# Ophiase/Stochastic-Vector-Oracle-Consensus

Measured on AMD Instinct MI355X. Metric: consensus updates/sec (N oracles x D dims, batched), higher is better.
Workload: dtype fp32; 1 GPU; model=svoc-consensus N=256 D=4096 streaming (f=32, constrained), global_batch=1024, seq_len=4096, parallelism=dp1, engine_mode=fast, storage=fp32, n_oracles=256, dimension=4096, n_failing=32, hip_graph=True, backend_world=1, stream_pool=89, independent_failing=False, transactional=False, fast_transactional=True, pipeline_chunks=2

## Files before the change

### csrc/include/svoc/slabdma.hpp

```cpp
#pragma once

#include <hip/hip_runtime.h>
#include <stdint.h>

#include "svoc/bufload.hpp"

namespace svoc {

typedef uint32_t u32x32_t __attribute__((ext_vector_type(32)));
typedef uint32_t u32x4_t __attribute__((ext_vector_type(4)));
struct RawRows {
  u32x32_t lo, hi;
  SVOC_DEV uint32_t at(int i) const { return i < 32 ? lo[i] : hi[i - 32]; }
};

template <int NSEG>
struct SlabDma {
  static constexpr int P = 64 / NSEG, CPR = P / 4, RPI = 64 / CPR;
  int vlane;
  int row0;
  int colb;
  SVOC_DEV SlabDma(int lane, int rowb) {
    const int j = lane / CPR;
    row0 = (j % NSEG) * 64 + j / NSEG;
    colb = (lane % CPR) * 16;
    vlane = row0 * rowb + colb;
  }
  SVOC_DEV int row_of(int k) const { return row0 + k * (RPI / NSEG); }
  static SVOC_DEV uint32_t lds_addr(uint32_t* region) {
    return (uint32_t)(uintptr_t)(__attribute__((address_space(3))) void*)region;
  }
  SVOC_DEV void issue(const BufDesc& rs, uint32_t* region, int rowb, int col0) const {
    const int vo = vlane + col0 * 4;
    const uint32_t lds0 = lds_addr(region);
#pragma unroll
    for (int k = 0; k < 16; ++k) {
      const uint32_t lds = lds0 + k * 1024u;
      int keep;
      asm volatile(
          "s_mov_b32 %0, m0\n\t"
          "s_mov_b32 m0, %3\n\t"
          "s_nop 0\n\t"
          "buffer_load_dwordx4 %1, %2, %4 offen lds\n\t"
          "s_mov_b32 m0, %0"
          : "=&s"(keep)
          : "v"(vo), "s"(rs.w), "s"(lds), "s"(k * (RPI / NSEG) * rowb)
          : "memory");
    }
  }
  template <class Sel, class OffB>
  SVOC_DEV void issue_mapped(const BufDesc& rs, const BufDesc& rb, uint32_t* region, int rowb, int col0, Sel sel,
                             OffB off_b) const {
    const int vo = vlane + col0 * 4;
    const uint32_t lds0 = lds_addr(region);
#pragma unroll
    for (int k = 0; k < 16; ++k) {
      const uint32_t lds = lds0 + k * 1024u;
      const uint32_t fb = sel(k);
      const int vb = off_b(k, fb);
      int keep;
      uint64_t sx;
      asm volatile(
          "s_mov_b32 %0, m0\n\t"
          "s_mov_b32 m0, %7\n\t"
          "s_mov_b64 %1, exec\n\t"
          "v_cmp_ne_u32 vcc, 0, %4\n\t"
          "s_nop 4\n\t"
          "s_andn2_b64 exec, %1, vcc\n\t"
          "s_nop 0\n\t"
          "buffer_load_dwordx4 %2, %5, %8 offen lds\n\t"
          "s_and_b64 exec, %1, vcc\n\t"
          "s_nop 0\n\t"
          "buffer_load_dwordx4 %3, %6, 0 offen lds\n\t"
          "s_mov_b64 exec, %1\n\t"
          "s_mov_b32 m0, %0"
          : "=&s"(keep), "=&s"(sx)
          : "v"(vo), "v"(vb), "v"(fb), "s"(rs.w), "s"(rb.w), "s"(lds), "s"(k * (RPI / NSEG) * rowb)
          : "vcc", "memory");
    }
  }
  template <class Sel, class OffB>
  SVOC_DEV void issue_mapped3(const BufDesc& rs, const BufDesc& rb, const BufDesc& rp, uint32_t* region, int rowb,
                              int col0, Sel sel, OffB off_b) const {
    const int vo = vlane + col0 * 4;
    const uint32_t lds0 = lds_addr(region);
#pragma unroll
    for (int k = 0; k < 16; ++k) {
      const uint32_t lds = lds0 + k * 1024u;
      const int fb = sel(k);
      const int vb = off_b(k);
      int keep;
      uint64_t sx, sp;
      asm volatile(
          "s_mov_b32 %0, m0\n\t"
          "s_mov_b32 m0, %9\n\t"
          "s_mov_b64 %1, exec\n\t"
          "v_cmp_gt_i32_e64 %2, 0, %5\n\t"
          "v_cmp_lt_i32 vcc, 0, %5\n\t"
          "s_nop 4\n\t"
          "s_and_b64 exec, %1, vcc\n\t"
          "s_nop 0\n\t"
          "buffer_load_dwordx4 %4, %7, 0 offen lds\n\t"
          "s_and_b64 exec, %1, %2\n\t"
          "s_or_b64 vcc, vcc, %2\n\t"
          "buffer_load_dwordx4 %4, %8, 0 offen lds\n\t"
          "s_andn2_b64 exec, %1, vcc\n\t"
          "s_nop 0\n\t"
          "buffer_load_dwordx4 %3, %6, %10 offen lds\n\t"
          "s_mov_b64 exec, %1\n\t"
          "s_mov_b32 m0, %0"
          : "=&s"(keep), "=&s"(sx), "=&s"(sp)
          : "v"(vo), "v"(vb), "v"(fb), "s"(rs.w), "s"(rb.w), "s"(rp.w), "s"(lds), "s"(k * (RPI / NSEG) * rowb)
          : "vcc", "memory");
    }
  }
};

}
```

### csrc/include/svoc/sortnet.hpp

```cpp
#pragma once

#include <hip/hip_runtime.h>
#include <stdint.h>

namespace svoc {

typedef unsigned short u16x2 __attribute__((ext_vector_type(2)));
typedef short s16x2 __attribute__((ext_vector_type(2)));

#define SVOC_DEV __device__ __forceinline__

SVOC_DEV u16x2 kmin(u16x2 a, u16x2 b) { return __builtin_elementwise_min(a, b); }
SVOC_DEV u16x2 kmax(u16x2 a, u16x2 b) { return __builtin_elementwise_max(a, b); }
SVOC_DEV uint32_t as_u32(u16x2 v) { return __builtin_bit_cast(uint32_t, v); }
SVOC_DEV u16x2 as_k(uint32_t v) { return __builtin_bit_cast(u16x2, v); }
SVOC_DEV uint32_t kmin(uint32_t a, uint32_t b) { return a < b ? a : b; }
SVOC_DEV uint32_t kmax(uint32_t a, uint32_t b) { return a < b ? b : a; }
SVOC_DEV uint32_t as_u32(uint32_t v) { return v; }
template <class K>
SVOC_DEV K key_from(uint32_t v) { return __builtin_bit_cast(K, v); }

SVOC_DEV u16x2 bf16x2_to_key(uint32_t raw) {
  u16x2 r = as_k(raw);
  u16x2 s = __builtin_bit_cast(u16x2, __builtin_bit_cast(s16x2, r) >> (short)15);
// ... 176 lines not shown
  m = 0u - (uint32_t)((k >> 4) & 1);
#pragma unroll
  for (int j = 0; j < 2; ++j) a[j] = blend(a[2 * j], a[2 * j + 1], m);
  m = 0u - (uint32_t)((k >> 5) & 1);
  return as_k(blend(a[0], a[1], m));
}

template <int NSEG, int P>
SVOC_DEV u16x2 group_select(const u16x2 (&r)[64], int rank, int lane) {
  const u16x2 v = reg_select(r, rank & 63);
  if constexpr (NSEG == 1) {
    return v;
  } else {
    const int owner = (rank >> 6) * P + (lane % P);
    return shfl_k(v, owner);
  }
}

template <int NSEG, int P, class K>
SVOC_DEV void middle_pair(const K (&r)[64], int seg, int lane, K& lo, K& hi) {
  if constexpr (NSEG == 1) {
    lo = r[31];
    hi = r[32];
  } else {
    constexpr int h = NSEG / 2;
    const int pw = lane % P;
    lo = shfl_k(r[63], (h - 1) * P + pw);
    hi = shfl_k(r[0], h * P + pw);
  }
}

template <int XM>
SVOC_DEV void xswap(uint32_t& x, uint32_t& y) {
  static_assert(XM == 16 || XM == 32, "lane-half exchange distance");
  if constexpr (XM == 32) {
    const auto t = __builtin_amdgcn_permlane32_swap(x, y, false, false);
    x = t[0];
    y = t[1];
  } else {
    const auto t = __builtin_amdgcn_permlane16_swap(x, y, false, false);
    x = t[0];
    y = t[1];
  }
}

template <int XM, class K>
SVOC_DEV void xhc_swap(K (&r)[64]) {
#pragma unroll
  for (int k = 0; k < 32; ++k) {
    uint32_t x = as_u32(r[2 * k]), y = as_u32(r[2 * k + 1]);
    xswap<XM>(x, y);
    y = ~y;
    const K lo = kmin(key_from<K>(x), key_from<K>(y)), hi = kmax(key_from<K>(x), key_from<K>(y));
    x = as_u32(lo);
    y = as_u32(hi);
    xswap<XM>(x, y);
    r[2 * k] = key_from<K>(x);
    r[2 * k + 1] = key_from<K>(y);
  }
}

template <int XM, class K>
SVOC_DEV void xhc_middle(const K (&r)[64], K& mx, K& mn) {
  mx = key_from<K>(0u);
  mn = key_from<K>(0xffffffffu);
#pragma unroll
  for (int k = 0; k < 32; ++k) {
    uint32_t x = as_u32(r[2 * k]), y = as_u32(r[2 * k + 1]);
    xswap<XM>(x, y);
    y = ~y;
    mx = kmax(mx, kmin(key_from<K>(x), key_from<K>(y)));
    mn = kmin(mn, kmax(key_from<K>(x), key_from<K>(y)));
  }
}

template <int NSEG>
SVOC_DEV uint32_t group_polarity(int seg) {
  if constexpr (NSEG == 2) return seg == 1 ? 0xffffffffu : 0u;
  else if constexpr (NSEG == 4) return (seg == 1 || seg == 2) ? 0xffffffffu : 0u;
  else return 0u;
}

template <int NSEG, class K>
SVOC_DEV void median_group(K (&r)[64], K& lo, K& hi) {
  sort_oem<64>(r);
  if constexpr (NSEG == 1) {
    lo = r[31];
    hi = r[32];
  } else {
    if constexpr (NSEG == 4) {
      xhc_swap<16>(r);
      merge64(r);
    }
    K mx, mn;
    xhc_middle<32>(r, mx, mn);
#pragma unroll
    for (int m = 16; m <= 32; m <<= 1) {
      if (NSEG == 2 && m == 16) continue;
      mx = kmax(mx, shfl_xor_k(mx, m));
      mn = kmin(mn, shfl_xor_k(mn, m));
    }
    lo = mx;
    hi = mn;
  }
}

template <int NSEG, int P, class K>
SVOC_DEV void median_group_wide(K (&r)[64], int seg, int lane, K& lo, K& hi) {
  static_assert(NSEG == 8 || NSEG == 16 || NSEG == 32 || NSEG == 64, "wide groups");
  sort_group<NSEG, P>(r, seg);
  middle_pair<NSEG, P>(r, seg, lane, lo, hi);
}


template <int XM, class K>
SVOC_DEV void xhc_pol(K (&r)[64], uint32_t iy, uint32_t ox, uint32_t oy) {
#pragma unroll
  for (int k = 0; k < 32; ++k) {
    uint32_t x = as_u32(r[2 * k]), y = as_u32(r[2 * k + 1]);
    xswap<XM>(x, y);
    y ^= iy;
    const K lo = kmin(key_from<K>(x), key_from<K>(y)), hi = kmax(key_from<K>(x), key_from<K>(y));
    x = as_u32(lo) ^ ox;
    y = as_u32(hi) ^ oy;
    xswap<XM>(x, y);
    r[2 * k] = key_from<K>(x);
    r[2 * k + 1] = key_from<K>(y);
  }
}

template <int H, class K>
SVOC_DEV void bitonic_top(const K (&r)[64], K (&out)[H]) {
  constexpr int KT = H - 1;
  static_assert(KT >= 2 && KT <= 32 && (KT & (KT - 1)) == 0, "H = 2^k + 1, at most 33");
  K t[64];
#pragma unroll
  for (int i = 0; i < 64; ++i) t[i] = r[i];
#pragma unroll
  for (int n = 64; n > 2 * KT; n >>= 1) {
#pragma unroll
    for (int i = 0; i < n / 2; ++i) t[i] = kmax(t[i], t[i + n / 2]);
  }
  K mx = kmin(t[0], t[KT]);
#pragma unroll
  for (int i = 0; i < KT; ++i) {
    const K a = t[i], b = t[i + KT];
    if (i) mx = kmax(mx, kmin(a, b));
    t[i] = kmax(a, b);
  }
#pragma unroll
  for (int j = KT / 2; j > 0; j >>= 1) {
#pragma unroll
    for (int i = 0; i < KT; ++i) {
      const int l = i ^ j;
      if (l > i) {
        const K a = t[i], b = t[l];
        t[i] = kmin(a, b);
        t[l] = kmax(a, b);
      }
    }
  }
  out[0] = mx;
#pragma unroll
  for (int i = 0; i < KT; ++i) out[i + 1] = t[i];
}

template <int NSEG, int P, int H, class K>
SVOC_DEV void window_group(K (&r)[64], int seg, int lane, K (&w)[NSEG == 1 ? 2 * H : H], K& lo, K& hi) {
  sort_oem<64>(r);
  if constexpr (NSEG == 1) {
#pragma unroll
    for (int m = 0; m < H; ++m) {
      w[m] = r[32 - H + m];
      w[H + m] = ~r[32 + H - 1 - m];
    }
    lo = r[31];
    hi = r[32];
  } else {
    if constexpr (NSEG == 2) {
      xhc_pol<32>(r, ~0u, 0u, ~0u);
    } else {
      xhc_swap<16>(r);
      merge64(r);
      xhc_pol<32>(r, ~0u, 0u, 0u);
      const uint32_t xm = seg >= 2 ? ~0u : 0u;
      xhc_pol<16>(r, 0u, xm, xm);
    }
    bitonic_top<H>(r, w);
    constexpr int slo = NSEG == 2 ? 0 : 1;
    const int pw = lane % P;
    lo = shfl_k(w[H - 1], slo * P + pw);
    hi = ~shfl_k(w[H - 1], (slo + 1) * P + pw);
  }
}



template <int XM, int L, class K>
SVOC_DEV void xhc_swap_n(K (&r)[L]) {
#pragma unroll
  for (int k = 0; k < L / 2; ++k) {
    uint32_t x = as_u32(r[2 * k]), y = as_u32(r[2 * k + 1]);
    xswap<XM>(x, y);
    y = ~y;
    const K lo = kmin(key_from<K>(x), key_from<K>(y)), hi = kmax(key_from<K>(x), key_from<K>(y));
    x = as_u32(lo);
    y = as_u32(hi);
    xswap<XM>(x, y);
    r[2 * k] = key_from<K>(x);
    r[2 * k + 1] = key_from<K>(y);
  }
}
template <int XM, int L, class K>
SVOC_DEV void xhc_pol_n(K (&r)[L], uint32_t iy, uint32_t ox, uint32_t oy) {
#pragma unroll
  for (int k = 0; k < L / 2; ++k) {
    uint32_t x = as_u32(r[2 * k]), y = as_u32(r[2 * k + 1]);
    xswap<XM>(x, y);
    y ^= iy;
    const K lo = kmin(key_from<K>(x), key_from<K>(y)), hi = kmax(key_from<K>(x), key_from<K>(y));
    x = as_u32(lo) ^ ox;
    y = as_u32(hi) ^ oy;
    xswap<XM>(x, y);
    r[2 * k] = key_from<K>(x);
    r[2 * k + 1] = key_from<K>(y);
  }
}
template <int L, class K>
SVOC_DEV void merge_n(K (&r)[L]) {
#pragma unroll
  for (int j = L / 2; j > 0; j >>= 1) {
#pragma unroll
    for (int i = 0; i < L; ++i) {
      const int l = i ^ j;
      if (l > i) {
        const K a = r[i], b = r[l];
        r[i] = kmin(a, b);
        r[l] = kmax(a, b);
      }
    }
  }
}
template <int H, int L, class K>
SVOC_DEV void bitonic_top_n(const K (&r)[L], K (&out)[H]) {
  constexpr int KT = H - 1;
  static_assert(2 * KT == L, "bitonic_top_n: L = 2 (H - 1)");
  K t[KT];
  K mx = kmin(r[0], r[KT]);
#pragma unroll
  for (int i = 0; i < KT; ++i) {
    const K a = r[i], b = r[i + KT];
    if (i) mx = kmax(mx, kmin(a, b));
    t[i] = kmax(a, b);
  }
#pragma unroll
  for (int j = KT / 2; j > 0; j >>= 1) {
#pragma unroll
    for (int i = 0; i < KT; ++i) {
      const int l = i ^ j;
      if (l > i) {
        const K a = t[i], b = t[l];
        t[i] = kmin(a, b);
        t[l] = kmax(a, b);
      }
    }
  }
  out[0] = mx;
#pragma unroll
  for (int i = 0; i < KT; ++i) out[i + 1] = t[i];
}

template <int P, int H, class K>
SVOC_DEV void window_group_pruned_sorted(K (&r)[64], int seg, int lane, K (&w)[H], K& lo, K& hi, bool& ok) {
  static_assert(H == 17, "pruned window: H = 17 (f <= 32 at N = 256)");
  const bool pol = seg == 1 || seg == 2;
  K dl = pol ? key_from<K>(~as_u32(r[48])) : r[15];
  K dh = pol ? key_from<K>(~as_u32(r[15])) : r[48];
  K k[32];
#pragma unroll
  for (int i = 0; i < 32; ++i) k[i] = r[16 + i];
  xhc_swap_n<16, 32>(k);
  merge_n<32>(k);
  xhc_pol_n<32, 32>(k, ~0u, 0u, 0u);
  const uint32_t xm = seg >= 2 ? ~0u : 0u;
  xhc_pol_n<16, 32>(k, 0u, xm, xm);
  bitonic_top_n<H, 32>(k, w);
  const int pw = lane % P;
  lo = shfl_k(w[H - 1], 1 * P + pw);
  hi = key_from<K>(~as_u32(shfl_k(w[H - 1], 2 * P + pw)));
  const K wlo = shfl_k(w[0], 1 * P + pw);
  const K whi = key_from<K>(~as_u32(shfl_k(w[0], 2 * P + pw)));
  dl = kmax(dl, key_from<K>(xor_lane_u32<16>(as_u32(dl))));
  dl = kmax(dl, key_from<K>(xor_lane_u32<32>(as_u32(dl))));
  dh = kmin(dh, key_from<K>(xor_lane_u32<16>(as_u32(dh))));
  dh = kmin(dh, key_from<K>(xor_lane_u32<32>(as_u32(dh))));
  ok = as_u32(kmax(dl, wlo)) == as_u32(wlo) && as_u32(kmin(dh, whi)) == as_u32(whi);
}
template <int P, int H, class K>
SVOC_DEV void window_group_pruned(K (&r)[64], int seg, int lane, K (&w)[H], K& lo, K& hi, bool& ok) {
  sort_oem<64>(r);
  window_group_pruned_sorted<P, H>(r, seg, lane, w, lo, hi, ok);
}

}
```

### csrc/kernels/consensus_fast_winf.hip

```cpp
#include <hip/hip_runtime.h>
#include <stdint.h>

#include <type_traits>
#include <utility>

#include "svoc/bufload.hpp"
#include "svoc/route.hpp"
#include "svoc/slabdma.hpp"
#include "svoc/rankmask.hpp"
#include "svoc/sortnet.hpp"
#include "svoc/status.hpp"
#include "svoc/verdict.hpp"

namespace svoc {

template <bool CONS>
SVOC_DEV uint32_t fkey(uint32_t raw) {
  if constexpr (CONS) return raw ^ 0x80000000u;
  else return f32_key(raw);
}
template <bool CONS>
SVOC_DEV float fkey_val(uint32_t k) {
  if constexpr (CONS) return __builtin_bit_cast(float, k ^ 0x80000000u);
  else return key_f32(k);
}
SVOC_DEV float u2f(uint32_t w) { return __builtin_bit_cast(float, w); }
SVOC_DEV uint32_t f2u(float v) { return __builtin_bit_cast(uint32_t, v); }

SVOC_DEV uint32_t winf_cand(uint32_t wt, uint32_t zt) {
  const uint32_t d = __builtin_elementwise_sub_sat(zt, wt);
  return wt | (__builtin_elementwise_min(d, 1u) - 1u);
}

struct MomKd {
  double n, in, k3, k4a, k4b, ik4c;
};
SVOC_DEV MomKd mom_kd(double n) {
  return MomKd{n, 1.0 / n, n / ((n - 1.0) * (n - 2.0)), n * (n + 1.0) / (n - 1.0), 3.0 * (n - 1.0) * (n - 1.0),
               1.0 / ((n - 2.0) * (n - 3.0))};
}
SVOC_DEV bool moments_from_sums_d(const MomKd& K, double t1, double t2, double t3, double t4, double& dl, float& sk,
                                  float& ku) {
#pragma clang fp contract(off)
  dl = t1 * K.in;
  const double e2 = t2 * K.in, e3 = t3 * K.in, e4 = t4 * K.in;
  const double mu2 = e2 - dl * dl;
  const double mu3 = e3 - 3.0 * dl * e2 + 2.0 * dl * dl * dl;
  const double mu4 = e4 - 4.0 * dl * e3 + 6.0 * dl * dl * e2 - 3.0 * dl * dl * dl * dl;
  sk = 0.f;
  ku = 0.f;
  if (!(mu2 > 0.0)) return false;
  const double r = 1.0 / mu2;
  sk = (float)(K.n * mu3 * r / sqrt(mu2) * K.k3);
  ku = (float)((K.n * mu4 * (r * r) * K.k4a - K.k4b) * K.ik4c);
  return true;
}

template <int MSK, int H>
SVOC_DEV void qr_halve(float (&part)[64], int lane) {
  if constexpr (MSK >= 1) {
    const bool up = (lane & MSK) != 0;
#pragma unroll
    for (int i = 0; i < H; ++i) {
      const float lo_v = part[i], hi_v = part[i + H];
      const float send = up ? lo_v : hi_v;
      const float keep = up ? hi_v : lo_v;
      part[i] = keep + xor_lane<MSK>(send);
    }
    qr_halve<MSK / 2, H / 2>(part, lane);
  }
}
template <bool MASKW, bool MASKROWS>
SVOC_DEV void qr_moments_regs(const RawRows& xs, int nvl, float c, uint32_t mw, f32x2 (&acc)[32],
                              f32x2& s1, f32x2& s2, f32x2& s3, f32x2& s4) {
#pragma clang fp contract(off)
#pragma unroll
  for (int m = 0; m < 32; ++m) {
    const uint32_t r0 = xs.at(2 * m), r1 = xs.at(2 * m + 1);
    const uint32_t w0 = MASKW ? r0 & mw : r0, w1 = MASKW ? r1 & mw : r1;
    f32x2 y = f32x2{u2f(w0), u2f(w1)} - f32x2{c, c};
    f32x2 q = y * y;
    acc[m] += q;
    if (MASKROWS) {
      const uint32_t m0 = lt_mask(2 * m, nvl), m1 = lt_mask(2 * m + 1, nvl);
      const float y0 = y.x, y1 = y.y, q0 = q.x, q1 = q.y;
      y = f32x2{fand(y0, m0), fand(y1, m1)};
      q = f32x2{fand(q0, m0), fand(q1, m1)};
    }
    s1 += y;
    s2 += q;
    s3 = __builtin_elementwise_fma(q, y, s3);
    s4 = __builtin_elementwise_fma(q, q, s4);
  }
}

template <int P>
SVOC_DEV void qr_keep(const f32x2 (&a)[32], int lane, float (&keep)[64 / P], bool add) {
  float part[64];
#pragma unroll
  for (int m = 0; m < 32; ++m) {
    part[2 * m] = a[m].x;
    part[2 * m + 1] = a[m].y;
  }
  qr_halve<P / 2, 32>(part, lane);
#pragma unroll
  for (int i = 0; i < 64 / P; ++i) keep[i] = add ? keep[i] + part[i] : part[i];
}

template <int P, int H, int WN>
SVOC_DEV bool try_pruned(uint32_t (&r)[64], int seg, int lane, uint32_t (&w)[WN], uint32_t& lo, uint32_t& hi,
                         uint32_t& e0, uint32_t& e63) {
  if constexpr (WN == H && H == 17) {
    bool ok;
    sort_oem<64>(r);
    e0 = r[0];
    e63 = r[63];
    window_group_pruned_sorted<P, H>(r, seg, lane, w, lo, hi, ok);
    return ok;
  } else {
    return false;
  }
}


template <int NSEG, int WAVES, int H, bool CONS, int MODE, bool FUSED = false, bool DEFER = false, bool WIDE = false>
__global__ __launch_bounds__(WAVES * 64) __attribute__((amdgpu_waves_per_eu(2))) void consensus_fast_winf_kernel(FastParams p) {
#pragma clang fp contract(off)
  constexpr int P = 64 / NSEG;
  constexpr int NPAD = 64 * NSEG;
  constexpr int W = WAVES * P;
  constexpr int NT = WAVES * 64;
  constexpr int KEEP = 64 / P;
  constexpr bool PASS1 = MODE != 2;
  __shared__ __attribute__((aligned(16))) uint32_t slab[PASS1 ? WAVES * 64 * 64 : 1];
  __shared__ __attribute__((aligned(16))) float qr_part[WAVES * NPAD];
  __shared__ float qr_lds[NPAD];
  __shared__ uint64_t relmask[4];
  __shared__ int urow[32];
  __shared__ float misc_f[2];
  __shared__ int misc_i[3];
  __shared__ uint32_t redo[128];
  __shared__ int smap[FUSED ? NPAD : 1];
  __shared__ int spend[DEFER ? NPAD : 1];
  __shared__ uint32_t badu[8];

  const int b = blockIdx.x;
  static_assert(!FUSED || (MODE == 0 && CONS), "fused streaming: whole constrained rounds");
  static_assert(!DEFER || FUSED, "deferred commit: a mode of the fused path");
  static_assert(!WIDE || (FUSED && !DEFER), "9-bit piece map: the fused path at 256 updates per instance");
  constexpr bool fused = FUSED;
  const int U = fused ? p.upd_per_inst : 0;
  if (p.active && !p.active[b]) {
    for (int t = threadIdx.x; t < U; t += WAVES * 64) p.upd_status[(int64_t)b * U + t] = ST_NOT_ACTIVE;
    return;
  }
  const int tid = threadIdx.x, lane = tid & 63, wave = __builtin_amdgcn_readfirstlane(tid >> 6);
  if (tid < 32) urow[tid] = 0;
  if (tid == 0) misc_i[2] = 0;
  if (tid < 128) redo[tid] = 0u;
  const int seg = lane / P, cw = lane % P;
  const int N = p.N, D = p.D;
  const int rowb = p.ld * 4;
  const float* inst = (const float*)p.values + (int64_t)b * p.inst_stride;
  const __amdgpu_buffer_rsrc_t rs = instance_rsrc(inst, (uint32_t)(N * rowb));
  const BufDesc rsd = buf_desc(inst, (uint32_t)(N * rowb));
  const int nslab = (D + W - 1) / W;
  const int Dc = 2 * p.work_pairs;
  const __amdgpu_buffer_rsrc_t ws = instance_rsrc(p.work + (int64_t)b * p.work_stride, (uint32_t)(p.work_stride * 4));
  const int MOM = 2 * H * Dc * 4;
  const int LST = MOM + 4 * Dc * 4;
  const int STG = Dc * kWinfStageCols * 4;
  const float* urows = fused ? p.upd_rows + (int64_t)b * U * D : inst;
  const uint32_t ubytes = fused ? (uint32_t)(U * D * 4) : 0u;
  const __amdgpu_buffer_rsrc_t rb = instance_rsrc(urows, ubytes);
  const BufDesc rbd = buf_desc(urows, ubytes);
  const float* prows = DEFER ? p.pend_rows + (int64_t)b * U * D : inst;
  const __amdgpu_buffer_rsrc_t rp = instance_rsrc(prows, DEFER ? ubytes : 0u);
  const BufDesc rpd = buf_desc(prows, DEFER ? ubytes : 0u);
  if constexpr (FUSED) {
    for (int t = tid; t < NPAD; t += NT) smap[t] = -1;
  }
  if constexpr (DEFER) {
    for (int t = tid; t < NPAD; t += NT) spend[t] = -1;
  }
  if (tid < 8) badu[tid] = 0u;
  __syncthreads();
  if (fused)
    for (int t = tid; t < U; t += NT) {
      const int64_t o = p.upd_oracle[(int64_t)b * U + t];
      if (o >= 0 && o < N) smap[o] = t;
      if constexpr (DEFER) {
        const int64_t q = p.pend_oracle[(int64_t)b * U + t];
        if (q >= 0 && q < N && p.pend_status[(int64_t)b * U + t] == ST_OK) spend[q] = t;
      }
    }
  __syncthreads();
  auto row_load = [&](int row, int cb) __attribute__((always_inline)) -> uint32_t {
    int u = -1;
    if constexpr (FUSED) u = __builtin_amdgcn_readfirstlane(smap[row]);
    if constexpr (DEFER) {
      const int q = __builtin_amdgcn_readfirstlane(spend[row]);
      if (u < 0 && q >= 0) return bload(rp, cb, q * D * 4);
    }
    return u >= 0 ? bload(rb, cb, u * D * 4) : bload(rs, cb, row * rowb);
  };
  auto bad_slot = [&](int u) __attribute__((always_inline)) { return (badu[u >> 5] >> (u & 31)) & 1u; };
  auto upd_out = [&](int st) __attribute__((always_inline)) {
    if (fused)
      for (int t = tid; t < U; t += NT) {
        int s = bad_slot(t) ? ST_INTERVAL_INPUT : st;
        const int64_t o = p.upd_oracle[(int64_t)b * U + t];
        if (o < 0 || o >= N) {
          s = ST_NOT_ORACLE;
          for (int d = 0; d < D; ++d) {
            const float v = urows[(int64_t)t * D + d];
            if (!(v >= 0.f && v <= 1.f)) {
              s = ST_INTERVAL_INPUT;
              break;
            }
          }
        }
        p.upd_status[(int64_t)b * U + t] = s;
      }
    if constexpr (DEFER) {
      for (int t = wave; t < U; t += WAVES) {
        const int64_t o = p.upd_oracle[(int64_t)b * U + t];
        if (o < 0 || o >= N || (st == ST_OK && !bad_slot(t))) continue;
        const int q = spend[o];
        if (q < 0) continue;
        float* dst = (float*)p.values + (int64_t)b * p.inst_stride + o * (int64_t)p.ld;
        for (int d = lane; d < D; d += 64) dst[d] = prows[(int64_t)q * D + d];
      }
    }
  };
  const int lo1 = (NPAD - N + 1) >> 1;
  const int nv = N - seg * 64;
  const int nl = N + lo1 - seg * 64;
  const uint32_t pol = group_polarity<NSEG>(seg);
  const uint32_t kp = 0x80000000u ^ pol;

  constexpr bool ACC64 = CONS;
  f32x2 acc[ACC64 ? 32 : 1];
#pragma unroll
  for (int i = 0; i < (ACC64 ? 32 : 1); ++i) acc[i] = f32x2{0.f, 0.f};
  float keep[KEEP];
#pragma unroll
  for (int i = 0; i < KEEP; ++i) keep[i] = 0.f;
  int net_fallbacks = 0;

  const int pass1_slabs = PASS1 ? nslab : 0;
  const SlabDma<NSEG> dma(lane, rowb);
  uint32_t* const region = slab + (PASS1 ? wave * 64 * 64 : 0);
  const uint32_t* const mine = region + (PASS1 ? seg * P + cw : 0);
  uint32_t pmap[FUSED ? (WIDE ? 5 : 4) : 1] = {};
  auto map_pieces = [&]() __attribute__((always_inline)) {
    if constexpr (FUSED) {
#pragma unroll
      for (int k = 0; k < 16; ++k) {
        const int row = dma.row_of(k);
        const int u = row < N ? smap[row] : -1;
        if (k % 4 == 0) pmap[k / 4] = 0u;
        if constexpr (DEFER) {
          const int q = row < N ? spend[row] : -1;
          pmap[k / 4] |= (uint32_t)(u >= 0 ? u + 1 : q >= 0 ? 0x80 | (q + 1) : 0) << (8 * (k % 4));
        } else if constexpr (WIDE) {
          if (k == 0) pmap[4] = 0u;
          pmap[k / 4] |= (uint32_t)((u + 1) & 0xff) << (8 * (k % 4));
          pmap[4] |= (uint32_t)((u + 1) >> 8) << k;
        } else
        pmap[k / 4] |= (uint32_t)(u + 1) << (8 * (k % 4));
      }
    }
  };
  auto issue_slab = [&](int s) __attribute__((always_inline)) {
    if constexpr (FUSED) {
      uint32_t pm[4] = {pmap[0], pmap[1], pmap[2], pmap[3]};
      asm volatile("" : "+v"(pm[0]), "+v"(pm[1]), "+v"(pm[2]), "+v"(pm[3]));
      int rowb_o = rowb, d4 = D * 4;
      asm volatile("" : "+s"(rowb_o), "+s"(d4));
      uint32_t* reg_o = region;
      asm volatile("" : "+s"(reg_o));
      int cbm = (s * W + wave * P) * 4 + dma.colb - d4;
      asm volatile("" : "+v"(cbm));
      if constexpr (DEFER)
        dma.issue_mapped3(
            rsd, rbd, rpd, reg_o, rowb_o, s * W + wave * P,
            [&](int k) { return (int)(pm[k / 4] << (24 - 8 * (k % 4))) >> 24; },
            [&](int k) { return (int)__umul24((pm[k / 4] >> (8 * (k % 4))) & 0x7fu, (unsigned)d4) + cbm; });
      else if constexpr (WIDE) {
        uint32_t ph = pmap[4];
        asm volatile("" : "+v"(ph));
        dma.issue_mapped(
            rsd, rbd, reg_o, rowb_o, s * W + wave * P,
            [&](int k) { return ((pm[k / 4] >> (8 * (k % 4))) & 0xffu) | (((ph >> k) & 1u) << 8); },
            [&](int, uint32_t fb) { return (int)__umul24(fb, (unsigned)d4) + cbm; });
      } else
      dma.issue_mapped(
          rsd, rbd, reg_o, rowb_o, s * W + wave * P,
          [&](int k) { return (pm[k / 4] >> (8 * (k % 4))) & 0xffu; },
          [&](int, uint32_t fb) { return (int)__umul24(fb, (unsigned)d4) + cbm; });
    } else {
      dma.issue(rsd, region, rowb, s * W + wave * P);
    }
  };
  for (int attempt = 0; attempt < 2; ++attempt) {
  if (fused) map_pieces();
  if (pass1_slabs > 0) issue_slab(0);
  auto slab_body = [&](auto full_c, int s) __attribute__((always_inline)) {
    constexpr bool FULL = decltype(full_c)::value;
    const int col = s * W + wave * P + cw;
    const bool vc = FULL || col < D;
    int nvl = nv, nll = nl;
    asm volatile("" : "+v"(nvl), "+v"(nll));
    float c1v;
    const uint32_t mW = vc ? 0xffffffffu : 0u;
    RawRows xs;
    __builtin_amdgcn_s_waitcnt(0x0F70);
    if constexpr (DEFER) {
      if (attempt == 0) {
        uint32_t pm[4] = {pmap[0], pmap[1], pmap[2], pmap[3]};
        asm volatile("" : "+v"(pm[0]), "+v"(pm[1]), "+v"(pm[2]), "+v"(pm[3]));
        int rowb_o = rowb;
        asm volatile("" : "+s"(rowb_o));
        const int c0 = s * W + wave * P;
        const int vo = dma.vlane + c0 * 4;
        const bool cvalid = FULL || c0 + (dma.colb >> 2) < D;
        const u32x4_t* piece = reinterpret_cast<const u32x4_t*>(region) + lane;
#pragma unroll
        for (int k0 = 0; k0 < 16; k0 += 8) {
          u32x4_t pc[8];
#pragma unroll
          for (int k = 0; k < 8; ++k) pc[k] = piece[(k0 + k) * 64];
#pragma unroll
          for (int k = 0; k < 8; ++k) asm volatile("" : "+v"(pc[k]));
#pragma unroll
          for (int k = k0; k < k0 + 8; ++k) {
            const int fb = (int)(pm[k / 4] << (24 - 8 * (k % 4))) >> 24;
            if (fb < 0 && cvalid)
              __builtin_amdgcn_raw_buffer_store_b128(pc[k - k0], rs, vo, k * (SlabDma<NSEG>::RPI / NSEG) * rowb_o, 0);
          }
        }
      }
    }
#pragma unroll
    for (int i = 0; i < 32; ++i) {
      xs.lo[i] = mine[i * 64];
      xs.hi[i] = mine[(i + 32) * 64];
    }
    __builtin_amdgcn_s_waitcnt(0xC07F);
    if (s + 1 < pass1_slabs) issue_slab(s + 1);
    constexpr bool IV_LATE = FUSED && FULL && CONS && NSEG == 4 && H == 17;
    auto mark_bad_rows = [&]() __attribute__((always_inline)) {
#pragma unroll
      for (int i = 0; i < 64; ++i) {
        const int row = seg * 64 + i;
        const uint32_t raw = xs.at(i);
        if (vc && row < N && !(raw <= 0x3f800000u || raw == 0x80000000u)) {
          int u = -1;
          if constexpr (FUSED) u = smap[row];
          if (u >= 0) atomicOr(&badu[u >> 5], 1u << (u & 31));
        }
      }
    };
    if (fused && !IV_LATE) {
      uint32_t mx = 0u;
#pragma unroll
      for (int i = 0; i < 64; i += 2) mx = __builtin_elementwise_max(mx, __builtin_elementwise_max(xs.at(i), xs.at(i + 1)));
      if (__ballot(mx > 0x3f800000u) != 0) mark_bad_rows();
    }
    {
      uint32_t r[64];
      auto build_keys = [&](uint32_t kpx) __attribute__((always_inline)) {
        if (FULL || N == NPAD) {
#pragma unroll
          for (int i = 0; i < 64; ++i) r[i] = CONS ? xs.at(i) ^ kpx : fkey<CONS>(xs.at(i)) ^ pol;
        } else {
#pragma unroll
          for (int i = 0; i < 64; ++i) {
            const uint32_t hi_m = ~lt_mask(i, nll);
            r[i] = ((fkey<CONS>(xs.at(i)) & (lt_mask(i, nvl) | hi_m)) | hi_m) ^ pol;
          }
        }
      };
      build_keys(kp);
      uint32_t klo, khi;
      if constexpr (CONS) {
        uint32_t wk[NSEG == 1 ? 2 * H : H];
        auto pruned_net = [&](auto full_c2) __attribute__((always_inline)) {
          if constexpr (NSEG == 4 && H == 17 && decltype(full_c2)::value) {
            uint32_t e0, e63;
            const bool ok = try_pruned<P, H>(r, seg, lane, wk, klo, khi, e0, e63);
            if constexpr (IV_LATE) {
              const uint32_t a = e0 ^ pol, bk = e63 ^ pol;
              const uint32_t tmin = __builtin_elementwise_min(a, bk), tmax = __builtin_elementwise_max(a, bk);
              if (__ballot(tmin < 0x80000000u || tmax > 0xbf800000u) != 0) mark_bad_rows();
            }
            if (__ballot(!ok) != 0) {
              ++net_fallbacks;
              uint32_t kpo = kp;
              asm volatile("" : "+v"(kpo));
              build_keys(kpo);
              window_group<NSEG, P, H>(r, seg, lane, wk, klo, khi);
            }
          } else {
            window_group<NSEG, P, H>(r, seg, lane, wk, klo, khi);
          }
        };
        pruned_net(full_c);
        if constexpr (NSEG == 1) {
#pragma unroll
          for (int m = 0; m < H; ++m) {
            bstore(ws, wk[m], col * 4, 2 * m * Dc * 4);
            bstore(ws, wk[H + m], (Dc + col) * 4, 2 * m * Dc * 4);
          }
        } else {
          constexpr int slo = NSEG == 2 ? 0 : 1;
          if (seg == slo || seg == slo + 1) {
            const int part = seg - slo;
#pragma unroll
            for (int m = 0; m < H; ++m) bstore(ws, wk[m], (part * Dc + col) * 4, 2 * m * Dc * 4);
          }
        }
      } else {
        median_group<NSEG>(r, klo, khi);
      }
      c1v = 0.5f * (fkey_val<CONS>(klo) + fkey_val<CONS>(khi));
    }
    if (seg == 0 && vc) p.c1[(int64_t)b * D + col] = c1v;
    const float cq = vc ? c1v : 0.f;
    f32x2 s1 = {0.f, 0.f}, s2 = s1, s3 = s1, s4 = s1;
    if constexpr (ACC64) {
      qr_moments_regs<!FULL, !FULL>(xs, nvl, cq, mW, acc, s1, s2, s3, s4);
    } else {
      f32x2 slab_acc[32];
#pragma unroll
      for (int i = 0; i < 32; ++i) slab_acc[i] = f32x2{0.f, 0.f};
      qr_moments_regs<!FULL, !FULL>(xs, nvl, cq, mW, slab_acc, s1, s2, s3, s4);
      qr_keep<P>(slab_acc, lane, keep, true);
    }
    float t1 = s1.x + s1.y, t2 = s2.x + s2.y, t3 = s3.x + s3.y, t4 = s4.x + s4.y;
    if constexpr (NSEG == 4) {
      t1 += xor_lane<16>(t1); t2 += xor_lane<16>(t2); t3 += xor_lane<16>(t3); t4 += xor_lane<16>(t4);
    }
    if constexpr (NSEG >= 2) {
      t1 += xor_lane<32>(t1); t2 += xor_lane<32>(t2); t3 += xor_lane<32>(t3); t4 += xor_lane<32>(t4);
    }
    if (seg == 0) {
      bstore(ws, f2u(t1), col * 4, MOM);
      bstore(ws, f2u(t2), col * 4, MOM + Dc * 4);
      bstore(ws, f2u(t3), col * 4, MOM + 2 * Dc * 4);
      bstore(ws, f2u(t4), col * 4, MOM + 3 * Dc * 4);
    }
  };
  if constexpr (PASS1) {
    const int nfull = N == NPAD ? min(D / W, pass1_slabs) : 0;
#pragma nounroll
    for (int s = 0; s < nfull; ++s) slab_body(std::true_type{}, s);
#pragma nounroll
    for (int s = nfull; s < pass1_slabs; ++s) slab_body(std::false_type{}, s);
  }
  if (!fused) break;
  __syncthreads();
  uint32_t anybad = 0u;
#pragma unroll
  for (int w = 0; w < 8; ++w) anybad |= badu[w];
  if (anybad == 0u || attempt == 1) break;
  if constexpr (FUSED) {
    for (int t = tid; t < NPAD; t += NT)
      if (smap[t] >= 0 && bad_slot(smap[t])) smap[t] = -1;
  }
  __syncthreads();
#pragma unroll
  for (int i = 0; i < (ACC64 ? 32 : 1); ++i) acc[i] = f32x2{0.f, 0.f};
#pragma unroll
  for (int i = 0; i < KEEP; ++i) keep[i] = 0.f;
  }

  if (net_fallbacks && lane == 0 && p.net_fallbacks) atomicAdd(p.net_fallbacks, (unsigned)net_fallbacks);
  {
    if constexpr (ACC64) qr_keep<P>(acc, lane, keep, false);
    int base = 0;
#pragma unroll
    for (int h = 32, msk = P / 2; msk >= 1; h >>= 1, msk >>= 1) base += (lane & msk) ? h : 0;
#pragma unroll
    for (int i = 0; i < KEEP; ++i) qr_part[wave * NPAD + seg * 64 + base + i] = keep[i];
  }
  __syncthreads();
  if (reduce_qr<NT, NPAD, WAVES, MODE>(p, b, N, tid, qr_part, qr_lds)) return;

  const int f = p.n_failing;
  const int R = N - f;
  if constexpr (CONS) {
    static_assert(WAVES >= 2, "rank keys in qr_part");
    rank_mask_nonneg<NT, NPAD>(qr_lds, reinterpret_cast<uint64_t*>(qr_part), N, R, tid, relmask);
  } else {
    rank_mask_general<NT, NPAD, 4>(qr_lds, N, R, tid, relmask);
  }
  __syncthreads();
  for (int t = tid; t < N; t += NT) {
    const int w = t >> 6;
    const uint64_t nr = ~relmask[w];
    if ((nr >> (t & 63)) & 1) {
      int cnt = __popcll(nr & ((1ull << (t & 63)) - 1));
      for (int v = 0; v < w; ++v) cnt += __popcll(~relmask[v]);
      if (cnt < 32) urow[cnt] = t;
    }
  }
  if (tid < 64) {
    double s_all = 0.0, s_rel = 0.0;
    for (int t = tid; t < N; t += 64) {
      const double q = (double)qr_lds[t];
      s_all += q;
      s_rel += ((relmask[t >> 6] >> (t & 63)) & 1) ? q : 0.0;
    }
#pragma unroll
    for (int o = 32; o >= 1; o >>= 1) {
      s_all += __shfl_xor(s_all, o);
      s_rel += __shfl_xor(s_rel, o);
    }
    if (tid == 0) {
      const RelF64 rel{CONS, rel_divisor<double>(p.legacy, p.rel_dim, D), (double)p.max_spread, N, R};
      const Verdict v = round_verdict(rel, s_all, s_rel, R, p.legacy);
      misc_f[0] = v.rel1;
      misc_f[1] = v.rel2;
      misc_i[0] = v.status;
      misc_i[1] = 0;
    }
  }
  __syncthreads();
  if (misc_i[0] != ST_OK) {
    if (tid == 0) p.status[b] = misc_i[0];
    upd_out(misc_i[0]);
    return;
  }

  if (CONS && !p.legacy) {
    const bool inwin = f + H <= N / 2;
    const int fr = first_reliable_row<4>(relmask);
    bool zv = false;
#pragma nounroll
    for (int base = wave * 64; base < D; base += WAVES * 64) {
      const int col = base + lane;
      const int pc = col < D ? col : D - 1;
      bool cand = col < D;
      if (inwin) {
        const uint32_t lo = bload(ws, pc * 4, 0), hi = ~bload(ws, (Dc + pc) * 4, 0);
        cand = cand && fkey_val<true>(lo) == fkey_val<true>(hi);
      }
      if (__ballot(cand)) {
        const float r0 = u2f(row_load(fr, pc * 4));
        for (int i = fr + 1; i < N; ++i) {
          if (!((relmask[i >> 6] >> (i & 63)) & 1)) continue;
          cand = cand && u2f(row_load(i, pc * 4)) == r0;
        }
        zv = zv || cand;
      }
    }
    if (zv) misc_i[1] = 1;
    __syncthreads();
    if (misc_i[1]) {
      if (tid == 0) p.status[b] = ST_ZERO_VARIANCE;
      upd_out(ST_ZERO_VARIANCE);
      return;
    }
  }
  if (CONS) {
    for (int t = tid; t < N; t += NT) {
      p.reliable[(int64_t)b * N + t] = (relmask[t >> 6] >> (t & 63)) & 1;
      p.qr[(int64_t)b * N + t] = qr_lds[t];
    }
  }

  const double n = (double)R;
  const MomKd mk = mom_kd(n);
  const int sh = H - 1 - (N / 2 - R / 2);
  const int64_t ob = (int64_t)b * D;
  bool zv = false;
  constexpr int NS = CONS ? 2 * H : 32;
  constexpr int NW = CONS ? H : 1;
  struct PBWords {
    uint32_t uw[NS];
    uint32_t wl[NW], wu[NW];
    uint32_t am[4];
    float c1c;
  };
  auto pb_load = [&](int base, PBWords& q) __attribute__((always_inline)) {
    const int col = base + lane;
    const int pc = col < D ? col : D - 1;
    const int vo = pc * 4;
    int shl = sh, fl = f;
    asm volatile("" : "+s"(shl), "+s"(fl));
    const int s0 = CONS ? shl : 0;
    const uint64_t realm = ((fl >= 64 ? ~0ull : (1ull << fl) - 1)) << s0;
    q.c1c = p.c1[ob + pc];
#pragma unroll
    for (int t = 0; t < NS; ++t) {
      const int row = t - s0;
      const bool real = (realm >> t) & 1;
      q.uw[t] = 0u;
      if (CONS || real) q.uw[t] = row_load(__builtin_amdgcn_readfirstlane(urow[real ? row : 0]), vo);
    }
    if constexpr (CONS) {
#pragma unroll
      for (int m = 0; m < H; ++m) {
        q.wl[m] = bload(ws, pc * 4, 2 * m * Dc * 4);
        q.wu[m] = ~bload(ws, (Dc + pc) * 4, 2 * m * Dc * 4);
      }
    }
#pragma unroll
    for (int k = 0; k < 4; ++k) q.am[k] = bload(ws, pc * 4, MOM + k * Dc * 4);
  };
  float* const o_lds = reinterpret_cast<float*>(slab);
  const bool ldso = CONS && PASS1 && D <= 4096;
  auto pb_col = [&](auto ldso_c, int base, const PBWords& cur) __attribute__((always_inline)) {
    constexpr bool LDSO = decltype(ldso_c)::value;
    const int col = base + lane;
    const float c1c = cur.c1c;
    int shl = sh, fl = f;
    asm volatile("" : "+s"(shl), "+s"(fl));
    const int s0 = CONS ? shl : 0;
    const uint64_t realm = ((fl >= 64 ? ~0ull : (1ull << fl) - 1)) << s0;
    const uint64_t lowm = (1ull << s0) - 1;
    float u1 = 0.f, u2 = 0.f, u3 = 0.f, u4 = 0.f;
#pragma unroll
    for (int t = 0; t < NS; ++t) {
      if ((realm >> t) & 1) {
        const float y = u2f(cur.uw[t]) - c1c;
        const float q = y * y;
        u1 += y;
        u2 += q;
        u3 = __builtin_fmaf(q, y, u3);
        u4 = __builtin_fmaf(q, q, u4);
      }
    }
    float cons_v = 0.f;
    if constexpr (CONS) {
      auto cands = [&](const auto& z) __attribute__((always_inline)) {
        uint32_t clo = ~0u, chi = ~0u;
#pragma unroll
        for (int m = 0; m < H; ++m) {
          const uint32_t wl = cur.wl[m], wu = cur.wu[m];
          clo = kmin(clo, winf_cand(wl, z(m)));
          if (m) chi = kmin(chi, winf_cand(wl, z(m - 1)));
          clo = kmin(clo, winf_cand(wu, z(2 * H - 1 - m)));
          chi = kmin(chi, winf_cand(wu, z(2 * H - 2 - m)));
        }
        cons_v = 0.5f * (fkey_val<true>(clo) + fkey_val<true>(chi));
      };
      constexpr int NF = H == 17 ? 32 : 8;
      if (s0 == 0 && fl == NF) {
        uint32_t z[NF];
#pragma unroll
        for (int t = 0; t < NF; ++t) z[t] = cur.uw[t] ^ 0x80000000u;
        sort_oem<NF>(z);
        cands([&](int t) __attribute__((always_inline)) { return t < NF ? z[t < NF ? t : 0] : ~0u; });
      } else {
        uint32_t z[64];
#pragma unroll
        for (int t = 0; t < 64; ++t) {
          if (t < 2 * H) {
            const uint32_t mreal = 0u - (uint32_t)((realm >> t) & 1);
            const uint32_t kx = (0x80000000u & mreal) | (~mreal & (0u - (uint32_t)(((~lowm) >> t) & 1)));
            z[t] = (cur.uw[t] & mreal) ^ kx;
          } else {
            z[t] = ~0u;
          }
        }
        sort_oem<64>(z);
        cands([&](int t) __attribute__((always_inline)) { return z[t]; });
      }
    }
    const double a1 = (double)u2f(cur.am[0]), a2 = (double)u2f(cur.am[1]);
    const double a3 = (double)u2f(cur.am[2]), a4 = (double)u2f(cur.am[3]);
    const double r1 = a1 - (double)u1, r2 = a2 - (double)u2, r3 = a3 - (double)u3, r4 = a4 - (double)u4;
    if (col < D) {
      const double rdl = r1 * mk.in, rmu2 = r2 * mk.in - rdl * rdl;
      const double wc = (double)p.win_cancel;
      const bool good = r2 > 0.0 && a2 <= wc * r2 && a4 <= wc * r4 && rdl * rdl <= 4.0 * rmu2;
      if constexpr (LDSO) {
        o_lds[col] = cons_v;
        o_lds[3 * D + col] = c1c;
      } else if (CONS) {
        p.consensus[ob + col] = cons_v;
        if (MODE == 0 && p.c1_out) p.c1_out[ob + col] = c1c;
      }
      if (good) {
        double dl;
        float sk, ku;
        const bool nz = moments_from_sums_d(mk, r1, r2, r3, r4, dl, sk, ku);
        if constexpr (LDSO) {
          o_lds[D + col] = p.legacy ? 0.f : sk;
          o_lds[2 * D + col] = p.legacy ? 0.f : ku;
        } else if (CONS) {
          p.skew[ob + col] = p.legacy ? 0.f : sk;
          p.kurt[ob + col] = p.legacy ? 0.f : ku;
        } else {
          stage_out(ws, STG, Dc, 0, col, (float)((double)c1c + dl));
          stage_out(ws, STG, Dc, 1, col, p.legacy ? 0.f : sk);
          stage_out(ws, STG, Dc, 2, col, p.legacy ? 0.f : ku);
          zv |= !nz;
        }
      } else if constexpr (LDSO) {
        atomicOr(&redo[col >> 5], 1u << (col & 31));
      } else {
        const int k = atomicAdd(&misc_i[2], 1);
        bstore(ws, (uint32_t)col, k * 4, LST);
      }
    }
  };
  if (ldso) {
    __builtin_amdgcn_s_waitcnt(0x0F70);
    PBWords cur;
    pb_load(wave * 64, cur);
#pragma nounroll
    for (int base = wave * 64; base < D; base += WAVES * 64) {
      PBWords nxt;
      if (base + WAVES * 64 < D) pb_load(base + WAVES * 64, nxt);
      asm volatile("" ::: "memory");
      pb_col(std::true_type{}, base, cur);
      cur = nxt;
    }
  } else {
#pragma nounroll
    for (int base = wave * 64; base < D; base += WAVES * 64) {
      PBWords cur;
      pb_load(base, cur);
      pb_col(std::false_type{}, base, cur);
    }
  }
  if (!CONS && zv && !p.legacy) misc_i[1] = 1;
  __syncthreads();
  auto cleanup_col = [&](int col) __attribute__((always_inline)) {
      const float cc = p.c1[ob + col];
      const float* xc = inst + col;
      float y[NSEG];
      float t1 = 0.f;
#pragma unroll
      for (int g = 0; g < NSEG; ++g) {
        const int i = g * 64 + lane;
        const bool use = i < N && ((relmask[g] >> lane) & 1);
        float xv = 0.f;
        if (use) {
          int u = -1, q = -1;
          if constexpr (FUSED) u = smap[i];
          if constexpr (DEFER) q = spend[i];
          xv = u >= 0 ? urows[(int64_t)u * D + col] : q >= 0 ? prows[(int64_t)q * D + col] : xc[(int64_t)i * p.ld];
        }
        y[g] = use ? xv - cc : 0.f;
        t1 += y[g];
      }
      t1 += xor_lane<1>(t1); t1 += xor_lane<2>(t1); t1 += xor_lane<4>(t1);
      t1 += xor_lane<8>(t1); t1 += xor_lane<16>(t1); t1 += xor_lane<32>(t1);
      const float mu = t1 / (float)R;
      float c1s = 0.f, t2 = 0.f, t3 = 0.f, t4 = 0.f;
#pragma unroll
      for (int g = 0; g < NSEG; ++g) {
        const int i = g * 64 + lane;
        const bool use = i < N && ((relmask[g] >> lane) & 1);
        const float d = use ? y[g] - mu : 0.f;
        const float q = d * d;
        c1s += d;
        t2 += q;
        t3 = fmaf(q, d, t3);
        t4 = fmaf(q, q, t4);
      }
      c1s += xor_lane<1>(c1s); t2 += xor_lane<1>(t2); t3 += xor_lane<1>(t3); t4 += xor_lane<1>(t4);
      c1s += xor_lane<2>(c1s); t2 += xor_lane<2>(t2); t3 += xor_lane<2>(t3); t4 += xor_lane<2>(t4);
      c1s += xor_lane<4>(c1s); t2 += xor_lane<4>(t2); t3 += xor_lane<4>(t3); t4 += xor_lane<4>(t4);
      c1s += xor_lane<8>(c1s); t2 += xor_lane<8>(t2); t3 += xor_lane<8>(t3); t4 += xor_lane<8>(t4);
      c1s += xor_lane<16>(c1s); t2 += xor_lane<16>(t2); t3 += xor_lane<16>(t3); t4 += xor_lane<16>(t4);
      c1s += xor_lane<32>(c1s); t2 += xor_lane<32>(t2); t3 += xor_lane<32>(t3); t4 += xor_lane<32>(t4);
      if (lane == 0) {
        double dl;
        float sk, ku;
        const bool nz = moments_from_sums_d(mk, c1s, t2, t3, t4, dl, sk, ku);
        if (CONS && ldso) {
          o_lds[D + col] = p.legacy ? 0.f : sk;
          o_lds[2 * D + col] = p.legacy ? 0.f : ku;
        } else if (CONS) {
          p.skew[ob + col] = p.legacy ? 0.f : sk;
          p.kurt[ob + col] = p.legacy ? 0.f : ku;
        } else {
          stage_out(ws, STG, Dc, 0, col, (float)((double)cc + (double)mu + dl));
          stage_out(ws, STG, Dc, 1, col, p.legacy ? 0.f : sk);
          stage_out(ws, STG, Dc, 2, col, p.legacy ? 0.f : ku);
          if (!nz && !p.legacy) misc_i[1] = 1;
// ... 121 lines not shown
```

Baseline: 590,200 consensus rounds/s.

## Remap four-segment lanes into quads and use DPP quad_perm sorting-network exchanges

For NSEG==4, the four segment lanes that share a column now sit in adjacent lanes (lane&3) instead of being 16 lanes apart. The slab DMA row/column mapping and the LDS reader addresses are rearranged to match, with a QUADBANK layout. The cross-segment merge, median and window networks now use DPP quad_perm exchanges instead of cross-lane xor shuffles over 16/32 lanes, and the moment reductions use xor 1/2. This aims to cut the cost of the cross-lane exchanges in the sort/select network. In exchange, the DMA layout changes, which may alter LDS bank conflicts and global coalescing.

```diff
diff --git a/csrc/include/svoc/slabdma.hpp b/csrc/include/svoc/slabdma.hpp
--- a/csrc/include/svoc/slabdma.hpp
+++ b/csrc/include/svoc/slabdma.hpp
@@ -14,17 +14,27 @@
   SVOC_DEV uint32_t at(int i) const { return i < 32 ? lo[i] : hi[i - 32]; }
 };
 
-template <int NSEG>
+template <int NSEG, bool QUADBANK = false>
 struct SlabDma {
+  static_assert(!QUADBANK || NSEG == 4, "QUADBANK: four lanes per column");
   static constexpr int P = 64 / NSEG, CPR = P / 4, RPI = 64 / CPR;
   int vlane;
   int row0;
   int colb;
   SVOC_DEV SlabDma(int lane, int rowb) {
-    const int j = lane / CPR;
-    row0 = (j % NSEG) * 64 + j / NSEG;
-    colb = (lane % CPR) * 16;
+    if constexpr (QUADBANK) {
+      row0 = ((lane & 6) << 5) + (lane >> 4);
+      colb = ((lane & 8) << 2) + ((lane & 1) << 4);
+    } else {
+      const int j = lane / CPR;
+      row0 = (j % NSEG) * 64 + j / NSEG;
+      colb = (lane % CPR) * 16;
+    }
     vlane = row0 * rowb + colb;
+  }
+  static SVOC_DEV int reader_word(int seg, int cw) {
+    if constexpr (QUADBANK) return 32 * (cw >> 3) + 8 * seg + 4 * ((cw >> 2) & 1) + (cw & 3);
+    else return seg * P + cw;
   }
   SVOC_DEV int row_of(int k) const { return row0 + k * (RPI / NSEG); }
   static SVOC_DEV uint32_t lds_addr(uint32_t* region) {
diff --git a/csrc/include/svoc/sortnet.hpp b/csrc/include/svoc/sortnet.hpp
--- a/csrc/include/svoc/sortnet.hpp
+++ b/csrc/include/svoc/sortnet.hpp
@@ -502,4 +502,113 @@
   window_group_pruned_sorted<P, H>(r, seg, lane, w, lo, hi, ok);
 }
 
-}
+template <int QP>
+SVOC_DEV uint32_t quad_perm(uint32_t v) {
+  return (uint32_t)__builtin_amdgcn_update_dpp(0, (int)v, QP, 0xF, 0xF, false);
+}
+template <int L>
+SVOC_DEV void qhc_first(uint32_t (&r)[L]) {
+#pragma unroll
+  for (int i = 0; i < L; ++i) {
+    const uint32_t t = ~quad_perm<0xB1>(r[i]);
+    r[i] = kmin(r[i], t);
+  }
+}
+SVOC_DEV uint32_t qhc_second_1(uint32_t x) {
+  const uint32_t t = ~quad_perm<0xC6>(x);
+  return kmin(quad_perm<0x6C>(x), t);
+}
+template <int L>
+SVOC_DEV void qhc_second(uint32_t (&r)[L]) {
+#pragma unroll
+  for (int i = 0; i < L; ++i) r[i] = qhc_second_1(r[i]);
+}
+template <int L>
+SVOC_DEV void qhc_last(const uint32_t (&r)[L], uint32_t (&o)[L]) {
+#pragma unroll
+  for (int i = 0; i < L / 2; ++i) {
+    const uint32_t a = r[i], b = r[L - 1 - i];
+    o[i] = kmax(a, quad_perm<0xB1>(b));
+    o[L - 1 - i] = kmax(b, quad_perm<0xB1>(a));
+  }
+}
+
+template <int H, int L>
+SVOC_DEV void bitonic_top_of(const uint32_t (&r)[L], uint32_t (&out)[H]) {
+  constexpr int KT = H - 1;
+  static_assert(KT >= 2 && (KT & (KT - 1)) == 0 && 2 * KT <= L && L <= 64, "H = 2^k + 1, 2 (H - 1) <= L");
+  uint32_t t[L];
+#pragma unroll
+  for (int i = 0; i < L; ++i) t[i] = r[i];
+#pragma unroll
+  for (int n = L; n > 2 * KT; n >>= 1) {
+#pragma unroll
+    for (int i = 0; i < n / 2; ++i) t[i] = kmax(t[i], t[i + n / 2]);
+  }
+  uint32_t h[2 * KT];
+#pragma unroll
+  for (int i = 0; i < 2 * KT; ++i) h[i] = t[i];
+  bitonic_top_n<H, 2 * KT>(h, out);
+}
+
+SVOC_DEV void median_group_quad(uint32_t (&r)[64], uint32_t& lo, uint32_t& hi) {
+  sort_oem<64>(r);
+  qhc_first<64>(r);
+  merge64(r);
+  uint32_t m = 0u;
+#pragma unroll
+  for (int i = 0; i < 64; ++i) m = kmax(m, qhc_second_1(r[i]));
+  m = kmax(m, quad_perm<0xB1>(m));
+  lo = quad_perm<0x00>(m);
+  hi = ~quad_perm<0xAA>(m);
+}
+
+template <int H, int WN>
+SVOC_DEV void window_group_quad(uint32_t (&r)[64], uint32_t (&w)[WN], uint32_t& lo, uint32_t& hi) {
+  static_assert(WN >= H, "window_group_quad: H keys per lane");
+  sort_oem<64>(r);
+  qhc_first<64>(r);
+  merge64(r);
+  qhc_second<64>(r);
+  uint32_t o[32];
+#pragma unroll
+  for (int i = 0; i < 16; ++i) {
+    const uint32_t a = r[i], b = r[63 - i], c = r[i + 32], d = r[31 - i];
+    o[i] = kmax(kmax(a, quad_perm<0xB1>(b)), kmax(c, quad_perm<0xB1>(d)));
+    o[31 - i] = kmax(kmax(d, quad_perm<0xB1>(c)), kmax(b, quad_perm<0xB1>(a)));
+  }
+  uint32_t t[H];
+  bitonic_top_of<H, 32>(o, t);
+#pragma unroll
+  for (int m = 0; m < H; ++m) w[m] = t[m];
+  lo = quad_perm<0x55>(t[H - 1]);
+  hi = ~quad_perm<0xAA>(t[H - 1]);
+}
+
+template <int H>
+SVOC_DEV void window_group_pruned_sorted_quad(uint32_t (&r)[64], int seg, uint32_t (&w)[H], uint32_t& lo,
+                                              uint32_t& hi, bool& ok) {
+  static_assert(H == 17, "pruned window: H = 17 (f <= 32 at N = 256)");
+  const bool pol = seg == 1 || seg == 2;
+  uint32_t dl = pol ? ~r[48] : r[15];
+  uint32_t dh = pol ? ~r[15] : r[48];
+  uint32_t k[32], o[32];
+#pragma unroll
+  for (int i = 0; i < 32; ++i) k[i] = r[16 + i];
+  qhc_first<32>(k);
+  merge_n<32>(k);
+  qhc_second<32>(k);
+  qhc_last<32>(k, o);
+  bitonic_top_n<H, 32>(o, w);
+  lo = quad_perm<0x55>(w[H - 1]);
+  hi = ~quad_perm<0xAA>(w[H - 1]);
+  const uint32_t wlo = quad_perm<0x55>(w[0]);
+  const uint32_t whi = ~quad_perm<0xAA>(w[0]);
+  dl = kmax(dl, quad_perm<0xB1>(dl));
+  dl = kmax(dl, quad_perm<0x4E>(dl));
+  dh = kmin(dh, quad_perm<0xB1>(dh));
+  dh = kmin(dh, quad_perm<0x4E>(dh));
+  ok = kmax(dl, wlo) == wlo && kmin(dh, whi) == whi;
+}
+
+}
diff --git a/csrc/kernels/consensus_fast_winf.hip b/csrc/kernels/consensus_fast_winf.hip
--- a/csrc/kernels/consensus_fast_winf.hip
+++ b/csrc/kernels/consensus_fast_winf.hip
@@ -56,18 +56,18 @@
   return true;
 }
 
-template <int MSK, int H>
-SVOC_DEV void qr_halve(float (&part)[64], int lane) {
+template <int MSK, int H, int SH>
+SVOC_DEV void qr_halve(float (&part)[64], int cw) {
   if constexpr (MSK >= 1) {
-    const bool up = (lane & MSK) != 0;
+    const bool up = (cw & MSK) != 0;
 #pragma unroll
     for (int i = 0; i < H; ++i) {
       const float lo_v = part[i], hi_v = part[i + H];
       const float send = up ? lo_v : hi_v;
       const float keep = up ? hi_v : lo_v;
-      part[i] = keep + xor_lane<MSK>(send);
-    }
-    qr_halve<MSK / 2, H / 2>(part, lane);
+      part[i] = keep + xor_lane<(MSK << SH)>(send);
+    }
+    qr_halve<MSK / 2, H / 2, SH>(part, cw);
   }
 }
 template <bool MASKW, bool MASKROWS>
@@ -94,28 +94,28 @@
   }
 }
 
-template <int P>
-SVOC_DEV void qr_keep(const f32x2 (&a)[32], int lane, float (&keep)[64 / P], bool add) {
+template <int P, int SH>
+SVOC_DEV void qr_keep(const f32x2 (&a)[32], int cw, float (&keep)[64 / P], bool add) {
   float part[64];
 #pragma unroll
   for (int m = 0; m < 32; ++m) {
     part[2 * m] = a[m].x;
     part[2 * m + 1] = a[m].y;
   }
-  qr_halve<P / 2, 32>(part, lane);
+  qr_halve<P / 2, 32, SH>(part, cw);
 #pragma unroll
   for (int i = 0; i < 64 / P; ++i) keep[i] = add ? keep[i] + part[i] : part[i];
 }
 
-template <int P, int H, int WN>
-SVOC_DEV bool try_pruned(uint32_t (&r)[64], int seg, int lane, uint32_t (&w)[WN], uint32_t& lo, uint32_t& hi,
+template <int H, int WN>
+SVOC_DEV bool try_pruned(uint32_t (&r)[64], int seg, uint32_t (&w)[WN], uint32_t& lo, uint32_t& hi,
                          uint32_t& e0, uint32_t& e63) {
   if constexpr (WN == H && H == 17) {
     bool ok;
     sort_oem<64>(r);
     e0 = r[0];
     e63 = r[63];
-    window_group_pruned_sorted<P, H>(r, seg, lane, w, lo, hi, ok);
+    window_group_pruned_sorted_quad<H>(r, seg, w, lo, hi, ok);
     return ok;
   } else {
     return false;
@@ -158,7 +158,10 @@
   if (tid < 32) urow[tid] = 0;
   if (tid == 0) misc_i[2] = 0;
   if (tid < 128) redo[tid] = 0u;
-  const int seg = lane / P, cw = lane % P;
+  constexpr bool QUAD = NSEG == 4;
+  constexpr int CWSH = QUAD ? 2 : 0;
+  const int seg = QUAD ? lane & 3 : lane / P, cw = QUAD ? lane >> 2 : lane % P;
+  const int qcol = QUAD ? cw : lane;
   const int N = p.N, D = p.D;
   const int rowb = p.ld * 4;
   const float* inst = (const float*)p.values + (int64_t)b * p.inst_stride;
@@ -249,9 +252,10 @@
   int net_fallbacks = 0;
 
   const int pass1_slabs = PASS1 ? nslab : 0;
-  const SlabDma<NSEG> dma(lane, rowb);
+  using Dma = SlabDma<NSEG, QUAD && H == 17>;
+  const Dma dma(lane, rowb);
   uint32_t* const region = slab + (PASS1 ? wave * 64 * 64 : 0);
-  const uint32_t* const mine = region + (PASS1 ? seg * P + cw : 0);
+  const uint32_t* const mine = region + (PASS1 ? Dma::reader_word(seg, cw) : 0);
   uint32_t pmap[FUSED ? (WIDE ? 5 : 4) : 1] = {};
   auto map_pieces = [&]() __attribute__((always_inline)) {
     if constexpr (FUSED) {
@@ -337,15 +341,21 @@
           for (int k = k0; k < k0 + 8; ++k) {
             const int fb = (int)(pm[k / 4] << (24 - 8 * (k % 4))) >> 24;
             if (fb < 0 && cvalid)
-              __builtin_amdgcn_raw_buffer_store_b128(pc[k - k0], rs, vo, k * (SlabDma<NSEG>::RPI / NSEG) * rowb_o, 0);
+              __builtin_amdgcn_raw_buffer_store_b128(pc[k - k0], rs, vo, k * (Dma::RPI / NSEG) * rowb_o, 0);
           }
         }
       }
     }
+    const uint32_t* rd = mine;
+    if constexpr (QUAD) {
+      int lq = lane;
+      asm volatile("" : "+v"(lq));
+      rd = region + Dma::reader_word(lq & 3, lq >> 2);
+    }
 #pragma unroll
     for (int i = 0; i < 32; ++i) {
-      xs.lo[i] = mine[i * 64];
-      xs.hi[i] = mine[(i + 32) * 64];
+      xs.lo[i] = rd[i * 64];
+      xs.hi[i] = rd[(i + 32) * 64];
     }
     __builtin_amdgcn_s_waitcnt(0xC07F);
     if (s + 1 < pass1_slabs) issue_slab(s + 1);
@@ -389,7 +399,7 @@
         auto pruned_net = [&](auto full_c2) __attribute__((always_inline)) {
           if constexpr (NSEG == 4 && H == 17 && decltype(full_c2)::value) {
             uint32_t e0, e63;
-            const bool ok = try_pruned<P, H>(r, seg, lane, wk, klo, khi, e0, e63);
+            const bool ok = try_pruned<H>(r, seg, wk, klo, khi, e0, e63);
             if constexpr (IV_LATE) {
               const uint32_t a = e0 ^ pol, bk = e63 ^ pol;
               const uint32_t tmin = __builtin_elementwise_min(a, bk), tmax = __builtin_elementwise_max(a, bk);
@@ -400,8 +410,10 @@
               uint32_t kpo = kp;
               asm volatile("" : "+v"(kpo));
               build_keys(kpo);
-              window_group<NSEG, P, H>(r, seg, lane, wk, klo, khi);
+              window_group_quad<H>(r, wk, klo, khi);
             }
+          } else if constexpr (QUAD) {
+            window_group_quad<H>(r, wk, klo, khi);
           } else {
             window_group<NSEG, P, H>(r, seg, lane, wk, klo, khi);
           }
@@ -422,7 +434,8 @@
           }
         }
       } else {
-        median_group<NSEG>(r, klo, khi);
+        if constexpr (QUAD) median_group_quad(r, klo, khi);
+        else median_group<NSEG>(r, klo, khi);
       }
       c1v = 0.5f * (fkey_val<CONS>(klo) + fkey_val<CONS>(khi));
     }
@@ -436,13 +449,13 @@
 #pragma unroll
       for (int i = 0; i < 32; ++i) slab_acc[i] = f32x2{0.f, 0.f};
       qr_moments_regs<!FULL, !FULL>(xs, nvl, cq, mW, slab_acc, s1, s2, s3, s4);
-      qr_keep<P>(slab_acc, lane, keep, true);
+      qr_keep<P, CWSH>(slab_acc, qcol, keep, true);
     }
     float t1 = s1.x + s1.y, t2 = s2.x + s2.y, t3 = s3.x + s3.y, t4 = s4.x + s4.y;
-    if constexpr (NSEG == 4) {
-      t1 += xor_lane<16>(t1); t2 += xor_lane<16>(t2); t3 += xor_lane<16>(t3); t4 += xor_lane<16>(t4);
-    }
-    if constexpr (NSEG >= 2) {
+    if constexpr (QUAD) {
+      t1 += xor_lane<1>(t1); t2 += xor_lane<1>(t2); t3 += xor_lane<1>(t3); t4 += xor_lane<1>(t4);
+      t1 += xor_lane<2>(t1); t2 += xor_lane<2>(t2); t3 += xor_lane<2>(t3); t4 += xor_lane<2>(t4);
+    } else if constexpr (NSEG == 2) {
       t1 += xor_lane<32>(t1); t2 += xor_lane<32>(t2); t3 += xor_lane<32>(t3); t4 += xor_lane<32>(t4);
     }
     if (seg == 0) {
@@ -478,10 +491,10 @@
 
   if (net_fallbacks && lane == 0 && p.net_fallbacks) atomicAdd(p.net_fallbacks, (unsigned)net_fallbacks);
   {
-    if constexpr (ACC64) qr_keep<P>(acc, lane, keep, false);
+    if constexpr (ACC64) qr_keep<P, CWSH>(acc, qcol, keep, false);
     int base = 0;
 #pragma unroll
-    for (int h = 32, msk = P / 2; msk >= 1; h >>= 1, msk >>= 1) base += (lane & msk) ? h : 0;
+    for (int h = 32, msk = P / 2; msk >= 1; h >>= 1, msk >>= 1) base += (qcol & msk) ? h : 0;
 #pragma unroll
     for (int i = 0; i < KEEP; ++i) qr_part[wave * NPAD + seg * 64 + base + i] = keep[i];
   }
```

Result: no change. 595,900 consensus rounds/s (median of 6 runs) (+1.0%).
